# facebookresearch/hyperreel

Hardware: NVIDIA H100
Metric: Mrays/s at 65k-ray x 32-sample batch (higher is better)
Workload: dtype f32 (sample net bf16x3 split on wgmma, fp32 accumulate)

## Files before the change

### hyperreel_b200/csrc/hr_mlp_tc2.cu

```cuda
#include <cuda.h>
#include <cuda_bf16.h>

#include <cstdio>
#include <cstdlib>
#include <cstring>

#include "hr_encode.cuh"
#include "hr_handle.h"
#include "hr_tc_prims.cuh"

namespace hr {

namespace tc2 {
using namespace tc;

constexpr int NSTAGE = 4;
constexpr int STAGE_BYTES = 8192;
constexpr int KSTEP_BYTES = 4096;
constexpr int CONSUMERS = 2;
constexpr int NTHREADS = (CONSUMERS + 1) * 128;
constexpr int PRODUCER_REGS = 40;
constexpr int CONSUMER_REGS = 232;
static_assert(128 * PRODUCER_REGS + CONSUMERS * 128 * CONSUMER_REGS <= 65536, "register file");

constexpr int A_BYTES = 16 * KSTEP_BYTES;
constexpr int OFF_AHI = 0;
constexpr int OFF_ALO = OFF_AHI + A_BYTES;
constexpr int X_BYTES = 4 * KSTEP_BYTES;
constexpr int OFF_X = OFF_ALO + A_BYTES;
constexpr int OFF_B = OFF_X + 2 * X_BYTES;
constexpr int OFF_BAR = OFF_B + CONSUMERS * NSTAGE * STAGE_BYTES;
constexpr int SMEM_BYTES = OFF_BAR + 128;
static_assert(SMEM_BYTES <= 232448, "shared memory budget");

constexpr int BAR_FULL = 0;
constexpr int BAR_EMPTY = BAR_FULL + CONSUMERS * NSTAGE;
static_assert((BAR_EMPTY + CONSUMERS * NSTAGE) * 8 <= 128, "barrier block");

constexpr int NB_RET = 3;
constexpr int NB_WR = 5;
constexpr int NB_XW = 7;
constexpr int NB_XR = 9;

}

template <int W, bool SAVE, bool NARROW>
__global__ void __launch_bounds__(tc2::NTHREADS, 1)
mlp_tc2_kernel(const __grid_constant__ hr_config cfg, const __grid_constant__ MlpTcPack pk, const float* __restrict__ rays,
               float* __restrict__ heads, long long n_rays, float* __restrict__ rays_copy, const TrainSave sv) {
  using namespace tc2;
  constexpr int WH = W / 2;
  constexpr int NACC = WH / 2;
  constexpr int NK = W / 16;
  constexpr int NKH = NK / 2;
  constexpr int IMG_BYTES = WH * 64;
  constexpr int KPS = STAGE_BYTES / IMG_BYTES;
  static_assert(KPS * IMG_BYTES == STAGE_BYTES && NKH % KPS == 0 && NK * KSTEP_BYTES <= A_BYTES, "pass width");
  extern __shared__ __align__(128) uint8_t smem[];
  const uint32_t sbase = smem_u32(smem);
  const int tid = threadIdx.x, warp = tid >> 5, lane = tid & 31;
  auto bar = [&](int slot) -> uint32_t { return sbase + OFF_BAR + slot * 8; };

  {
    const char* w = reinterpret_cast<const char*>(pk.wpack);
    const long long lines = pk.wpack_bytes >> 7;
    for (long long i = (long long)blockIdx.x * NTHREADS + tid; i < lines; i += (long long)gridDim.x * NTHREADS)
      asm volatile("prefetch.global.L2 [%0];" ::"l"(w + i * 128));
  }
  for (int i = tid; i < (2 * X_BYTES) / 16; i += NTHREADS)
    reinterpret_cast<uint4*>(smem + OFF_X)[i] = make_uint4(0u, 0u, 0u, 0u);
  if (tid == 0) {
    for (int s = 0; s < CONSUMERS * NSTAGE; ++s) { mbar_init(bar(BAR_FULL + s), 1); mbar_init(bar(BAR_EMPTY + s), 1); }
    asm volatile("fence.mbarrier_init.release.cluster;" ::: "memory");
  }
  __syncthreads();

  const long long n_tiles = (n_rays + BM - 1) / BM;
  const int n_passes = pk.n_passes;
  const long long n_iters = ((long long)blockIdx.x < n_tiles) ? (n_tiles - 1 - blockIdx.x) / gridDim.x + 1 : 0;

  if (warp >= CONSUMERS * 4) {
    setmaxnreg_dec<PRODUCER_REGS>();
    const int g = warp - CONSUMERS * 4;
    if (g < CONSUMERS && lane == 0) {
      const long long half_bytes = pk.wpack_bytes / CONSUMERS;
      const int n_stages = (int)(half_bytes / STAGE_BYTES);
      const uint32_t full0 = bar(BAR_FULL + g * NSTAGE), empty0 = bar(BAR_EMPTY + g * NSTAGE);
      const uint32_t ring = sbase + OFF_B + (uint32_t)(g * NSTAGE * STAGE_BYTES);
      uint32_t stage = 0, phase = 0;
      for (long long iter = 0; iter < n_iters; ++iter) {
        const uint8_t* src = reinterpret_cast<const uint8_t*>(pk.wpack) + g * half_bytes;
        for (int i = 0; i < n_stages; ++i) {
          mbar_wait(empty0 + stage * 8, phase ^ 1);
          mbar_expect_tx(full0 + stage * 8, STAGE_BYTES);
          bulk_g2s(ring + stage * STAGE_BYTES, src, STAGE_BYTES, full0 + stage * 8);
          src += STAGE_BYTES;
          if (++stage == NSTAGE) { stage = 0; phase ^= 1; }
        }
      }
    }
    return;
  }

  setmaxnreg_inc<CONSUMER_REGS>();
  const int wg = warp >> 2;
  const int wt = tid & 127;
  const int rowq = (warp & 3) * 16 + (lane >> 2);
  const int q2 = (lane & 3) * 2;
  const int col0 = wg * WH;
  const int in_chunks = pk.in_chunks;
  const int L = cfg.mlp_layers;
  const uint32_t x_lo_off = (uint32_t)(2 * in_chunks * KSTEP_BYTES);
  const uint32_t full0 = bar(BAR_FULL + wg * NSTAGE), empty0 = bar(BAR_EMPTY + wg * NSTAGE);
  const uint32_t ring = sbase + OFF_B + (uint32_t)(wg * NSTAGE * STAGE_BYTES);
  const bool vec_ok = ((reinterpret_cast<uintptr_t>(rays) | reinterpret_cast<uintptr_t>(rays_copy)) & 15) == 0;
  int x_last = 0;
  for (int p = 0; p < n_passes; ++p)
    if (pk.passes[p].first_chunk == 0) x_last = p;
  uint32_t stage = 0, phase = 0;
  int pend = -1;

  float acc[2][NACC];

  auto stage_begin = [&]() {
    mbar_wait(full0 + stage * 8, phase);
    wgmma_fence();
    acc_fence(acc[0]);
    acc_fence(acc[1]);
  };
  auto stage_end = [&]() {
    wgmma_commit();
    acc_fence(acc[0]);
    acc_fence(acc[1]);
    wgmma_wait<1>();
    if (pend >= 0 && wt == 0) mbar_arrive(empty0 + pend * 8);
    pend = (int)stage;
    if (++stage == NSTAGE) { stage = 0; phase ^= 1; }
  };
  auto b_img = [&](int sub) -> uint32_t { return ring + stage * STAGE_BYTES + (uint32_t)sub * IMG_BYTES; };
  auto kstep = [&](uint32_t a, uint32_t a_lo, uint32_t b, uint32_t scale) {
    const uint64_t bh = gmma_desc(b, WH * 16, 128), bl = gmma_desc(b + WH * 32, WH * 16, 128);
    const uint64_t ah0 = gmma_desc(a, 2048, 128), ah1 = gmma_desc(a + 1024, 2048, 128);
    const uint64_t al0 = gmma_desc(a + a_lo, 2048, 128), al1 = gmma_desc(a + a_lo + 1024, 2048, 128);
    wgmma_ss(acc[0], ah0, bh, scale);
    wgmma_ss(acc[1], ah1, bh, scale);
    wgmma_ss(acc[0], al0, bh, 1u);
    wgmma_ss(acc[1], al1, bh, 1u);
    wgmma_ss(acc[0], ah0, bl, 1u);
    wgmma_ss(acc[1], ah1, bl, 1u);
  };
  auto run_pass = [&](const TcPass& P, bool fresh, bool x_ret, bool ret) {
    int ki = 0;
    if (P.first_chunk == 0) {
      for (; ki < 2 * in_chunks; ki += KPS) {
        stage_begin();
#pragma unroll
        for (int sub = 0; sub < KPS; ++sub)
          kstep(sbase + OFF_X + (uint32_t)(ki + sub) * KSTEP_BYTES, x_lo_off, b_img(sub), (ki + sub) != 0 ? 1u : 0u);
        stage_end();
      }
    }
    if (P.first_chunk + P.n_chunks > in_chunks) {
      const uint32_t scale0 = ki != 0 ? 1u : 0u;
#pragma unroll
      for (int kk = 0; kk < NK; ++kk) {
        if (kk % KPS == 0) {
          if (fresh && kk == (wg == 0 ? NKH : 0)) {
            if (wg == 0) pair_arrive(NB_WR + 0);
            pair_wait(NB_WR + (wg ^ 1));
          }
          stage_begin();
        }
        kstep(sbase + OFF_AHI + (uint32_t)kk * KSTEP_BYTES, OFF_ALO - OFF_AHI, b_img(kk % KPS), kk != 0 ? 1u : scale0);
        if (kk % KPS == KPS - 1) {
          stage_end();
          if (x_ret && kk == KPS - 1) pair_arrive(NB_XR + wg);
          if (ret && wg == 1 && kk == NKH + KPS - 1) pair_arrive(NB_RET + 1);
        }
      }
    }
  };
  auto drain = [&]() {
    wgmma_wait<0>();
    acc_fence(acc[0]);
    acc_fence(acc[1]);
    if (pend >= 0 && wt == 0) mbar_arrive(empty0 + pend * 8);
    pend = -1;
  };
  const int st_row = (warp & 3) * 16 + 8 * ((lane >> 3) & 1) + (lane & 7);
  const uint32_t st_off = ks_slot(st_row, lane >> 4);
  auto store_hidden = [&](const float* bias, int layer, long long tile) {
#pragma unroll
    for (int kk = 0; kk < NKH; ++kk) {
      float2 b[2];
#pragma unroll
      for (int jj = 0; jj < 2; ++jj) b[jj] = __ldg(reinterpret_cast<const float2*>(bias + col0 + 8 * (2 * kk + jj) + q2));
#pragma unroll
      for (int m = 0; m < 2; ++m) {
        uint32_t hi[4], lo[4];
#pragma unroll
        for (int jj = 0; jj < 2; ++jj) {
          const int j = 2 * kk + jj, k = col0 + 8 * j + q2;
#pragma unroll
          for (int h = 0; h < 2; ++h) {
            float t0 = acc[m][4 * j + 2 * h] + b[jj].x, t1 = acc[m][4 * j + 2 * h + 1] + b[jj].y;
            t0 = fmaxf(t0, t0 * cfg.leaky_slope);
            t1 = fmaxf(t1, t1 * cfg.leaky_slope);
            split2(t0, t1, hi[2 * jj + h], lo[2 * jj + h]);
            if constexpr (SAVE) {
              const long long ray = tile * BM + 64 * m + rowq + 8 * h;
              if (ray < n_rays) *reinterpret_cast<float2*>(sv.act + layer * sv.act_stride + ray * W + k) = make_float2(t0, t1);
            }
          }
        }
        const uint32_t a = sbase + st_off + (uint32_t)m * 1024u + (uint32_t)(wg * NKH + kk) * KSTEP_BYTES;
        stmatrix_x4(a + OFF_AHI, hi);
        stmatrix_x4(a + OFF_ALO, lo);
      }
    }
  };
  auto encode = [&](long long tile, bool after_x) {
    if (after_x) pair_wait(NB_XR + (wg ^ 1));
    const int r = wg * 64 + (wt & 63), part = wt >> 6;
    const long long ray = tile * BM + r;
    auto put = [&](int k, float val) {
      if constexpr (SAVE) {
        if (ray < n_rays) sv.enc[ray * sv.ld_enc + k] = val;
      }
      const __nv_bfloat16 hi = __float2bfloat16_rn(val);
      const __nv_bfloat16 lo = __float2bfloat16_rn(val - __bfloat162float(hi));
      const uint32_t off = (uint32_t)(k >> 4) * KSTEP_BYTES + ks_slot(r, (k >> 3) & 1) + (uint32_t)(k & 7) * 2u;
      *reinterpret_cast<__nv_bfloat16*>(smem + OFF_X + off) = hi;
      *reinterpret_cast<__nv_bfloat16*>(smem + OFF_X + x_lo_off + off) = lo;
    };
    if (ray < n_rays) {
      float rbuf[16];
      const float* src = rays + ray * cfg.c_in;
      if (cfg.c_in == 8 && vec_ok) {
        const float4 a = *reinterpret_cast<const float4*>(src), b = *reinterpret_cast<const float4*>(src + 4);
        rbuf[0] = a.x; rbuf[1] = a.y; rbuf[2] = a.z; rbuf[3] = a.w; rbuf[4] = b.x; rbuf[5] = b.y; rbuf[6] = b.z; rbuf[7] = b.w;
        if (rays_copy != nullptr && part == 0) {
          float4* dst = reinterpret_cast<float4*>(rays_copy + ray * 8);
          dst[0] = a; dst[1] = b;
        }
      } else {
        for (int i = 0; i < cfg.c_in; ++i) rbuf[i] = src[i];
        if (rays_copy != nullptr && part == 0)
          for (int i = 0; i < cfg.c_in; ++i) rays_copy[ray * cfg.c_in + i] = rbuf[i];
      }
      encode_ray_features(cfg, rbuf, part, 2, put);
      if constexpr (SAVE) {
        if (part == 0)
          for (int k = cfg.mlp_in; k < sv.ld_enc; ++k) sv.enc[ray * sv.ld_enc + k] = 0.0f;
      }
    } else if (part == 0) {
      for (int k = 0; k < cfg.mlp_in; ++k) put(k, 0.0f);
    }
    fence_async_smem();
    wg_sync(1 + wg);
    pair_arrive(NB_XW + wg);
  };

  for (long long iter = 0; iter < n_iters; ++iter) {
    const long long tile = iter * gridDim.x + blockIdx.x;
    const bool more = iter + 1 < n_iters;
    if (iter == 0) encode(tile, false);
    pair_wait(NB_XW + (wg ^ 1));
    for (int p = 0; p < n_passes; ++p) {
      const TcPass& P = pk.passes[p];
      const bool reads_a = P.first_chunk + P.n_chunks > in_chunks;
      const bool hidden = p < L - 1;
      const bool ret = reads_a && (hidden || (p == n_passes - 1 && more));
      const bool x_ret = p == x_last && more;
      run_pass(P, reads_a && P.wait_a != 0, x_ret, ret);
      drain();
      if (x_ret && !reads_a) pair_arrive(NB_XR + wg);
      if (ret && wg == 0) pair_arrive(NB_RET + 0);
      if (hidden) {
        wg_sync(1 + wg);
        if (p > 0 || iter > 0) pair_wait(NB_RET + (wg ^ 1));
        store_hidden(pk.bias + P.bias_off, p, tile);
        fence_async_smem();
        wg_sync(1 + wg);
        if (wg == 1) pair_arrive(NB_WR + 1);
      } else {
        const float* bias = pk.bias + P.bias_off;
        if constexpr (SAVE) {
#pragma unroll
          for (int m = 0; m < 2; ++m)
#pragma unroll
            for (int h = 0; h < 2; ++h) {
              const long long ray = tile * BM + 64 * m + rowq + 8 * h;
              if (ray >= n_rays) continue;
              float* row = heads + ray * cfg.mlp_out;
#pragma unroll
              for (int j = 0; j < WH / 8; ++j) {
                const int c = col0 + 8 * j + q2;
                if (P.out_col0 + c < cfg.mlp_out) {
                  const float2 b = __ldg(reinterpret_cast<const float2*>(bias + c));
                  const int c0 = P.out_col0 + c, c1 = c0 + 1, S = cfg.n_samples;
                  row[(c0 % S) * cfg.head_stride + c0 / S] = acc[m][4 * j + 2 * h] + b.x;
                  if (c1 < cfg.mlp_out) row[(c1 % S) * cfg.head_stride + c1 / S] = acc[m][4 * j + 2 * h + 1] + b.y;
                }
              }
            }
        } else if constexpr (NARROW) {
          const bool pairs = (cfg.mlp_out % 2) == 0 && (reinterpret_cast<uintptr_t>(heads) & 7) == 0;
#pragma unroll
          for (int j = 0; j < WH / 8; ++j) {
            const int c = col0 + 8 * j + q2, c0 = P.out_col0 + c;
            const float2 b = __ldg(reinterpret_cast<const float2*>(bias + c));
#pragma unroll
            for (int m = 0; m < 2; ++m)
#pragma unroll
              for (int h = 0; h < 2; ++h) {
                const long long ray = tile * BM + 64 * m + rowq + 8 * h;
                if (ray >= n_rays || c0 >= cfg.mlp_out) continue;
                float* dst = heads + ray * cfg.mlp_out + c0;
                const float v0 = acc[m][4 * j + 2 * h] + b.x, v1 = acc[m][4 * j + 2 * h + 1] + b.y;
                if (pairs) {
                  *reinterpret_cast<float2*>(dst) = make_float2(v0, v1);
                } else {
                  dst[0] = v0;
                  if (c0 + 1 < cfg.mlp_out) dst[1] = v1;
                }
              }
          }
        } else {
          const bool odd = (lane & 1) != 0;
#pragma unroll
          for (int jp = 0; jp < WH / 16; ++jp) {
            const int j = 2 * jp, c = col0 + 8 * j + q2;
            const float2 b0 = __ldg(reinterpret_cast<const float2*>(bias + c));
            const float2 b1 = __ldg(reinterpret_cast<const float2*>(bias + c + 8));
#pragma unroll
            for (int m = 0; m < 2; ++m)
#pragma unroll
              for (int h = 0; h < 2; ++h) {
                const float2 v0 = make_float2(acc[m][4 * j + 2 * h] + b0.x, acc[m][4 * j + 2 * h + 1] + b0.y);
                const float2 v1 = make_float2(acc[m][4 * j + 4 + 2 * h] + b1.x, acc[m][4 * j + 4 + 2 * h + 1] + b1.y);
                const float2 send = odd ? v0 : v1;
                const float2 recv = make_float2(__shfl_xor_sync(0xffffffffu, send.x, 1), __shfl_xor_sync(0xffffffffu, send.y, 1));
                const int c4 = odd ? c + 6 : c;
                const long long ray = tile * BM + 64 * m + rowq + 8 * h;
                if (ray < n_rays && P.out_col0 + c4 < cfg.mlp_out)
                  *reinterpret_cast<float4*>(heads + ray * cfg.mlp_out + P.out_col0 + c4) =
                      odd ? make_float4(recv.x, recv.y, v1.x, v1.y) : make_float4(v0.x, v0.y, recv.x, recv.y);
              }
          }
        }
      }
      if (x_ret) encode(tile + gridDim.x, true);
    }
  }
}

int pack_mlp_tc2(SampleNet& net, const float* const* w_dev, const float* const* b_dev, cudaStream_t st) {
  const hr_config& c = net.cfg;
  MlpTcPack& pk = net.tc;
  size_t& alloc_bytes = net.tc_alloc_bytes;
  int& alloc_bias = net.tc_alloc_bias;
  const int W = c.mlp_width;
  if (W != 128 && W != 256) return hr_fail("tensor-core sample net: hidden width must be 128 or 256 (got %d)", W);
  if (c.mlp_in > 64) return hr_fail("tensor-core sample net: encoded input wider than 64 features (%d)", c.mlp_in);
  const int in_chunks = (c.mlp_in + 31) / 32;
  const int L = c.mlp_layers;
  MlpTcPack np_{};
  np_.in_chunks = in_chunks;
  int np = 0, bias_off = 0;
  size_t bytes = 0;
  for (int l = 0; l < L; ++l) {
    const bool last = (l == L - 1);
    const int out = last ? c.mlp_out : W;
    const int n_parts = (out + W - 1) / W;
    for (int part = 0; part < n_parts; ++part) {
      if (np >= HR_TC_MAX_PASSES) return hr_fail("tensor-core sample net: too many passes (%d output columns)", c.mlp_out);
      TcPass& P = np_.passes[np++];
      const bool reads_input = (l == 0 || l == c.mlp_skip);
      P.layer = l;
      P.n = W;
      P.first_chunk = reads_input ? 0 : in_chunks;
      P.n_chunks = (l == 0) ? in_chunks : (W / 32 + (reads_input ? in_chunks : 0));
      P.bias_off = bias_off;
      P.is_final = last ? 1 : 0;
      P.out_col0 = part * W;
      P.wait_a = (part == 0) ? 1 : 0;
      bias_off += P.n;
      bytes += (size_t)P.n_chunks * 2 * P.n * 64;
    }
  }
  np_.n_passes = np;
  np_.bias_count = bias_off;
  np_.wpack_bytes = (long long)bytes;
  if (alloc_bytes != bytes || alloc_bias != bias_off || !pk.wpack) {
    if (pk.wpack) cudaFree(const_cast<void*>(pk.wpack));
    if (pk.bias) cudaFree(const_cast<float*>(pk.bias));
    pk.wpack = nullptr; pk.bias = nullptr;
    alloc_bytes = 0; alloc_bias = 0;
    void* wp = nullptr; float* bp = nullptr;
    cudaError_t e = cudaMalloc(&wp, bytes);
    if (e != cudaSuccess) return hr_fail("cudaMalloc(tc weights %zu): %s", bytes, cudaGetErrorString(e));
    e = cudaMalloc((void**)&bp, (size_t)bias_off * sizeof(float));
    if (e != cudaSuccess) { cudaFree(wp); return hr_fail("cudaMalloc(tc bias): %s", cudaGetErrorString(e)); }
    np_.wpack = wp; np_.bias = bp;
    alloc_bytes = bytes; alloc_bias = bias_off;
    for (int narrow = 0; narrow < 2 && e == cudaSuccess; ++narrow) {
      auto kern = (W == 256) ? (narrow ? mlp_tc2_kernel<256, false, true> : mlp_tc2_kernel<256, false, false>)
                             : (narrow ? mlp_tc2_kernel<128, false, true> : mlp_tc2_kernel<128, false, false>);
      e = cudaFuncSetAttribute(kern, cudaFuncAttributeMaxDynamicSharedMemorySize, tc2::SMEM_BYTES);
    }
    if (e != cudaSuccess) return hr_fail("cudaFuncSetAttribute(mlp_tc2_kernel): %s", cudaGetErrorString(e));
  } else {
    np_.wpack = pk.wpack; np_.bias = pk.bias;
  }
  pk = np_;
  uint8_t* wp = (uint8_t*)const_cast<void*>(pk.wpack);
  float* bp = const_cast<float*>(pk.bias);
  const int WH = W / 2;
  for (int half = 0; half < 2; ++half) {
    size_t off = (size_t)half * (bytes / 2);
    for (int p = 0; p < np; ++p) {
      const TcPass& P = pk.passes[p];
      const int l = P.layer;
      const bool last = (l == L - 1), skip = (l == c.mlp_skip), first = (l == 0);
      const int in_src = first ? c.mlp_in : (skip ? c.mlp_in + W : W);
      launch_pack_tc_pass(w_dev[l], b_dev[l], wp + off, bp + P.bias_off + half * WH, WH, P.first_chunk, P.n_chunks, in_src,
                          c.mlp_in, skip ? 1 : 0, in_chunks, last ? c.mlp_out : W, last ? c.n_samples : 0, c.head_stride,
                          P.out_col0 + half * WH, st);
      off += (size_t)P.n_chunks * 2 * WH * 64;
    }
  }
  cudaError_t e = cudaGetLastError();
  if (e != cudaSuccess) return hr_fail("tc pack launch failed: %s", cudaGetErrorString(e));
  return 0;
}

void free_mlp_tc2(SampleNet& net) {
  if (net.tc.wpack) cudaFree(const_cast<void*>(net.tc.wpack));
  if (net.tc.bias) cudaFree(const_cast<float*>(net.tc.bias));
  net.tc.wpack = nullptr; net.tc.bias = nullptr;
  net.tc_alloc_bytes = 0; net.tc_alloc_bias = 0;
}

cudaError_t launch_mlp_tc2(const hr_config& cfg, const MlpTcPack& pk, const float* rays, float* heads, long long n, int num_sms,
                           cudaStream_t stream, float* rays_copy) {
  long long tiles = (n + tc::BM - 1) / tc::BM;
  int grid = (int)(tiles < num_sms ? tiles : num_sms);
  if (grid < 1) grid = 1;
  const bool narrow = (cfg.mlp_out % 4) != 0 || ((uintptr_t)heads % 16) != 0;
  auto kern = cfg.mlp_width == 256 ? (narrow ? mlp_tc2_kernel<256, false, true> : mlp_tc2_kernel<256, false, false>)
                                   : (narrow ? mlp_tc2_kernel<128, false, true> : mlp_tc2_kernel<128, false, false>);
  if (cfg.mlp_width != 256 && cfg.mlp_width != 128) return cudaErrorInvalidValue;
  kern<<<grid, tc2::NTHREADS, tc2::SMEM_BYTES, stream>>>(cfg, pk, rays, heads, n, rays_copy, TrainSave{});
  return cudaGetLastError();
}

cudaError_t launch_mlp_tc2_train(const hr_config& cfg, const MlpTcPack& pk, const float* rays, float* heads, long long n,
                                 int num_sms, cudaStream_t stream, const TrainSave& sv) {
  long long tiles = (n + tc::BM - 1) / tc::BM;
  int grid = (int)(tiles < num_sms ? tiles : num_sms);
  if (grid < 1) grid = 1;
  auto kern = cfg.mlp_width == 256 ? mlp_tc2_kernel<256, true, false> : mlp_tc2_kernel<128, true, false>;
  if (cfg.mlp_width != 256 && cfg.mlp_width != 128) return cudaErrorInvalidValue;
  cudaError_t e = cudaFuncSetAttribute(kern, cudaFuncAttributeMaxDynamicSharedMemorySize, tc2::SMEM_BYTES);
  if (e != cudaSuccess) return e;
  kern<<<grid, tc2::NTHREADS, tc2::SMEM_BYTES, stream>>>(cfg, pk, rays, heads, n, nullptr, sv);
  return cudaGetLastError();
}

}
```

### hyperreel_b200/csrc/hr_tc_prims.cuh

```cuda
#pragma once
#include <cuda.h>
#include <cuda_bf16.h>
#include <stdint.h>

namespace hr {
namespace tc {

constexpr int BM = 128;

__device__ __forceinline__ uint32_t smem_u32(const void* p) { return (uint32_t)__cvta_generic_to_shared(p); }

__device__ __forceinline__ void mbar_init(uint32_t bar, uint32_t count) {
  asm volatile("mbarrier.init.shared::cta.b64 [%0], %1;" ::"r"(bar), "r"(count) : "memory");
}
__device__ __forceinline__ void mbar_arrive(uint32_t bar) {
  asm volatile("{\n\t.reg .b64 st;\n\tmbarrier.arrive.shared::cta.b64 st, [%0];\n\t}" ::"r"(bar) : "memory");
}
__device__ __forceinline__ void mbar_expect_tx(uint32_t bar, uint32_t bytes) {
  asm volatile("{\n\t.reg .b64 st;\n\tmbarrier.arrive.expect_tx.shared::cta.b64 st, [%0], %1;\n\t}" ::"r"(bar), "r"(bytes)
               : "memory");
}
__device__ __forceinline__ void mbar_wait(uint32_t bar, uint32_t parity) {
  asm volatile(
      "{\n\t"
      ".reg .pred p;\n\t"
      "WAIT_LOOP:\n\t"
      "mbarrier.try_wait.parity.shared::cta.b64 p, [%0], %1;\n\t"
      "@p bra DONE;\n\t"
      "bra WAIT_LOOP;\n\t"
      "DONE:\n\t"
      "}" ::"r"(bar), "r"(parity)
      : "memory");
}
__device__ __forceinline__ void bulk_g2s(uint32_t dst, const void* src, uint32_t bytes, uint32_t bar) {
  asm volatile("cp.async.bulk.shared::cluster.global.mbarrier::complete_tx::bytes [%0], [%1], %2, [%3];" ::"r"(dst), "l"(src),
               "r"(bytes), "r"(bar)
               : "memory");
}
__device__ __forceinline__ void fence_async_smem() { asm volatile("fence.proxy.async.shared::cta;" ::: "memory"); }
__device__ __forceinline__ void wg_sync(int id) { asm volatile("bar.sync %0, 128;" ::"r"(id) : "memory"); }
__device__ __forceinline__ void pair_arrive(int id) { asm volatile("bar.arrive %0, 256;" ::"r"(id) : "memory"); }
__device__ __forceinline__ void pair_wait(int id) { asm volatile("bar.sync %0, 256;" ::"r"(id) : "memory"); }

__device__ __forceinline__ uint64_t gmma_desc(uint32_t saddr, uint32_t lbo_bytes, uint32_t sbo_bytes) {
  uint64_t d = 0;
  d |= (uint64_t)((saddr & 0x3FFFF) >> 4);
  d |= (uint64_t)((lbo_bytes >> 4) & 0x3FFF) << 16;
  d |= (uint64_t)((sbo_bytes >> 4) & 0x3FFF) << 32;
  return d;
}

__device__ __forceinline__ void wgmma_fence() { asm volatile("wgmma.fence.sync.aligned;" ::: "memory"); }
__device__ __forceinline__ void wgmma_commit() { asm volatile("wgmma.commit_group.sync.aligned;" ::: "memory"); }
template <int N>
__device__ __forceinline__ void wgmma_wait() {
  asm volatile("wgmma.wait_group.sync.aligned %0;" ::"n"(N) : "memory");
}
template <int N>
__device__ __forceinline__ void acc_fence(float (&d)[N]) {
#pragma unroll
  for (int i = 0; i < N; ++i) asm volatile("" : "+f"(d[i])::"memory");
}
template <int R>
__device__ __forceinline__ void setmaxnreg_dec() { asm volatile("setmaxnreg.dec.sync.aligned.u32 %0;" ::"n"(R)); }
template <int R>
__device__ __forceinline__ void setmaxnreg_inc() { asm volatile("setmaxnreg.inc.sync.aligned.u32 %0;" ::"n"(R)); }

__device__ __forceinline__ void wgmma_ss(float (&d)[32], uint64_t adesc, uint64_t bdesc, uint32_t accumulate) {
  asm volatile(
      "{\n\t"
      ".reg .pred p;\n\t"
      "setp.ne.b32 p, %34, 0;\n\t"
      "wgmma.mma_async.sync.aligned.m64n64k16.f32.bf16.bf16 "
      "{"
      "%0, %1, %2, %3, %4, %5, %6, %7, %8, %9, %10, %11, %12, %13, %14, %15, %16, %17, %18, %19, %20, %21, %22, "
      "%23, %24, %25, %26, %27, %28, %29, %30, %31"
      "}, %32, %33, p, 1, 1, 0, 0;\n\t"
      "}"
      : "+f"(d[0]), "+f"(d[1]), "+f"(d[2]), "+f"(d[3]), "+f"(d[4]), "+f"(d[5]), "+f"(d[6]), "+f"(d[7]),
        "+f"(d[8]), "+f"(d[9]), "+f"(d[10]), "+f"(d[11]), "+f"(d[12]), "+f"(d[13]), "+f"(d[14]), "+f"(d[15]),
        "+f"(d[16]), "+f"(d[17]), "+f"(d[18]), "+f"(d[19]), "+f"(d[20]), "+f"(d[21]), "+f"(d[22]), "+f"(d[23]),
        "+f"(d[24]), "+f"(d[25]), "+f"(d[26]), "+f"(d[27]), "+f"(d[28]), "+f"(d[29]), "+f"(d[30]), "+f"(d[31])
      : "l"(adesc), "l"(bdesc), "r"(accumulate));
}

__device__ __forceinline__ void wgmma_ss(float (&d)[64], uint64_t adesc, uint64_t bdesc, uint32_t accumulate) {
  asm volatile(
      "{\n\t"
      ".reg .pred p;\n\t"
      "setp.ne.b32 p, %66, 0;\n\t"
      "wgmma.mma_async.sync.aligned.m64n128k16.f32.bf16.bf16 "
      "{"
      "%0, %1, %2, %3, %4, %5, %6, %7, %8, %9, %10, %11, %12, %13, %14, %15, %16, %17, %18, %19, %20, %21, %22, "
      "%23, %24, %25, %26, %27, %28, %29, %30, %31, %32, %33, %34, %35, %36, %37, %38, %39, %40, %41, %42, %43, "
      "%44, %45, %46, %47, %48, %49, %50, %51, %52, %53, %54, %55, %56, %57, %58, %59, %60, %61, %62, %63"
      "}, %64, %65, p, 1, 1, 0, 0;\n\t"
      "}"
      : "+f"(d[0]), "+f"(d[1]), "+f"(d[2]), "+f"(d[3]), "+f"(d[4]), "+f"(d[5]), "+f"(d[6]), "+f"(d[7]),
        "+f"(d[8]), "+f"(d[9]), "+f"(d[10]), "+f"(d[11]), "+f"(d[12]), "+f"(d[13]), "+f"(d[14]), "+f"(d[15]),
        "+f"(d[16]), "+f"(d[17]), "+f"(d[18]), "+f"(d[19]), "+f"(d[20]), "+f"(d[21]), "+f"(d[22]), "+f"(d[23]),
        "+f"(d[24]), "+f"(d[25]), "+f"(d[26]), "+f"(d[27]), "+f"(d[28]), "+f"(d[29]), "+f"(d[30]), "+f"(d[31]),
        "+f"(d[32]), "+f"(d[33]), "+f"(d[34]), "+f"(d[35]), "+f"(d[36]), "+f"(d[37]), "+f"(d[38]), "+f"(d[39]),
        "+f"(d[40]), "+f"(d[41]), "+f"(d[42]), "+f"(d[43]), "+f"(d[44]), "+f"(d[45]), "+f"(d[46]), "+f"(d[47]),
        "+f"(d[48]), "+f"(d[49]), "+f"(d[50]), "+f"(d[51]), "+f"(d[52]), "+f"(d[53]), "+f"(d[54]), "+f"(d[55]),
        "+f"(d[56]), "+f"(d[57]), "+f"(d[58]), "+f"(d[59]), "+f"(d[60]), "+f"(d[61]), "+f"(d[62]), "+f"(d[63])
      : "l"(adesc), "l"(bdesc), "r"(accumulate));
}

__device__ __forceinline__ void stmatrix_x4(uint32_t addr, const uint32_t (&r)[4]) {
  asm volatile("stmatrix.sync.aligned.m8n8.x4.shared.b16 [%0], {%1, %2, %3, %4};" ::"r"(addr), "r"(r[0]), "r"(r[1]), "r"(r[2]),
               "r"(r[3])
               : "memory");
}

__device__ __forceinline__ uint32_t ks_slot(int row, int kg) { return (uint32_t)((kg * 16 + (row >> 3)) * 128 + (row & 7) * 16); }

__device__ __forceinline__ void split2(float x0, float x1, uint32_t& hi, uint32_t& lo) {
  __nv_bfloat162 hh = __floats2bfloat162_rn(x0, x1);
  __nv_bfloat162 ll = __floats2bfloat162_rn(x0 - __low2float(hh), x1 - __high2float(hh));
  hi = *reinterpret_cast<uint32_t*>(&hh);
  lo = *reinterpret_cast<uint32_t*>(&ll);
}

}

void launch_pack_tc_pass(const float* W, const float* b, uint8_t* dst, float* bias_dst, int n, int first_chunk, int n_chunks,
                         int in_src, int mlp_in, int is_skip, int in_chunks, int out_rows, int perm_S, int perm_stride,
                         int out_col0, cudaStream_t st);
}
```

Baseline: 155.3.

## Move ray encoding into dedicated encoder warps of the producer warpgroup

Result: faster. 157.6, median of 6 (+1.5%).

```diff
diff --git a/hyperreel_b200/csrc/hr_mlp_tc2.cu b/hyperreel_b200/csrc/hr_mlp_tc2.cu
--- a/hyperreel_b200/csrc/hr_mlp_tc2.cu
+++ b/hyperreel_b200/csrc/hr_mlp_tc2.cu
@@ -19,9 +19,11 @@
 constexpr int KSTEP_BYTES = 4096;
 constexpr int CONSUMERS = 2;
 constexpr int NTHREADS = (CONSUMERS + 1) * 128;
-constexpr int PRODUCER_REGS = 40;
-constexpr int CONSUMER_REGS = 232;
-static_assert(128 * PRODUCER_REGS + CONSUMERS * 128 * CONSUMER_REGS <= 65536, "register file");
+constexpr int ENCODERS = 64;
+constexpr int PRODUCER_REGS = 56;
+constexpr int CONSUMER_REGS = 224;
+constexpr int LAUNCH_REGS = 168;
+static_assert(128 * PRODUCER_REGS + CONSUMERS * 128 * CONSUMER_REGS <= NTHREADS * LAUNCH_REGS, "register file");
 
 constexpr int A_BYTES = 16 * KSTEP_BYTES;
 constexpr int OFF_AHI = 0;
@@ -39,9 +41,51 @@
 
 constexpr int NB_RET = 3;
 constexpr int NB_WR = 5;
-constexpr int NB_XW = 7;
-constexpr int NB_XR = 9;
-
+constexpr int NB_XFULL = 7;
+constexpr int NB_XFREE = 9;
+constexpr int XFULL_THREADS = ENCODERS + 128;
+constexpr int XFREE_THREADS = CONSUMERS * 128 + ENCODERS;
+
+}
+
+template <bool SAVE>
+__device__ __forceinline__ void encode_row(const hr_config& cfg, const float* __restrict__ rays, long long n_rays,
+                                           float* __restrict__ rays_copy, const TrainSave& sv, uint8_t* smem,
+                                           uint32_t x_lo_off, bool vec_ok, long long tile, int r) {
+  using namespace tc2;
+  const long long ray = tile * BM + r;
+  auto put = [&](int k, float val) {
+    if constexpr (SAVE) {
+      if (ray < n_rays) sv.enc[ray * sv.ld_enc + k] = val;
+    }
+    const __nv_bfloat16 hi = __float2bfloat16_rn(val);
+    const __nv_bfloat16 lo = __float2bfloat16_rn(val - __bfloat162float(hi));
+    const uint32_t off = (uint32_t)(k >> 4) * KSTEP_BYTES + ks_slot(r, (k >> 3) & 1) + (uint32_t)(k & 7) * 2u;
+    *reinterpret_cast<__nv_bfloat16*>(smem + OFF_X + off) = hi;
+    *reinterpret_cast<__nv_bfloat16*>(smem + OFF_X + x_lo_off + off) = lo;
+  };
+  if (ray < n_rays) {
+    float rbuf[16];
+    const float* src = rays + ray * cfg.c_in;
+    if (cfg.c_in == 8 && vec_ok) {
+      const float4 a = *reinterpret_cast<const float4*>(src), b = *reinterpret_cast<const float4*>(src + 4);
+      rbuf[0] = a.x; rbuf[1] = a.y; rbuf[2] = a.z; rbuf[3] = a.w; rbuf[4] = b.x; rbuf[5] = b.y; rbuf[6] = b.z; rbuf[7] = b.w;
+      if (rays_copy != nullptr) {
+        float4* dst = reinterpret_cast<float4*>(rays_copy + ray * 8);
+        dst[0] = a; dst[1] = b;
+      }
+    } else {
+      for (int i = 0; i < cfg.c_in; ++i) rbuf[i] = src[i];
+      if (rays_copy != nullptr)
+        for (int i = 0; i < cfg.c_in; ++i) rays_copy[ray * cfg.c_in + i] = rbuf[i];
+    }
+    encode_ray_features(cfg, rbuf, 0, 1, put);
+    if constexpr (SAVE) {
+      for (int k = cfg.mlp_in; k < sv.ld_enc; ++k) sv.enc[ray * sv.ld_enc + k] = 0.0f;
+    }
+  } else {
+    for (int k = 0; k < cfg.mlp_in; ++k) put(k, 0.0f);
+  }
 }
 
 template <int W, bool SAVE, bool NARROW>
@@ -79,10 +123,23 @@
   const int n_passes = pk.n_passes;
   const long long n_iters = ((long long)blockIdx.x < n_tiles) ? (n_tiles - 1 - blockIdx.x) / gridDim.x + 1 : 0;
 
+  const int in_chunks = pk.in_chunks;
+  const uint32_t x_lo_off = (uint32_t)(2 * in_chunks * KSTEP_BYTES);
   if (warp >= CONSUMERS * 4) {
     setmaxnreg_dec<PRODUCER_REGS>();
     const int g = warp - CONSUMERS * 4;
-    if (g < CONSUMERS && lane == 0) {
+    if (g >= CONSUMERS) {
+      const int et = tid - (NTHREADS - ENCODERS);
+      const bool vec_ok = ((reinterpret_cast<uintptr_t>(rays) | reinterpret_cast<uintptr_t>(rays_copy)) & 15) == 0;
+      for (long long iter = 0; iter < n_iters; ++iter) {
+        const long long tile = iter * gridDim.x + blockIdx.x;
+        if (iter > 0) bar_sync_n(NB_XFREE, XFREE_THREADS);
+        for (int r = et; r < BM; r += ENCODERS)
+          encode_row<SAVE>(cfg, rays, n_rays, rays_copy, sv, smem, x_lo_off, vec_ok, tile, r);
+        fence_async_smem();
+        for (int c = 0; c < CONSUMERS; ++c) bar_arrive_n(NB_XFULL + c, XFULL_THREADS);
+      }
+    } else if (lane == 0) {
       const long long half_bytes = pk.wpack_bytes / CONSUMERS;
       const int n_stages = (int)(half_bytes / STAGE_BYTES);
       const uint32_t full0 = bar(BAR_FULL + g * NSTAGE), empty0 = bar(BAR_EMPTY + g * NSTAGE);
@@ -108,12 +165,9 @@
   const int rowq = (warp & 3) * 16 + (lane >> 2);
   const int q2 = (lane & 3) * 2;
   const int col0 = wg * WH;
-  const int in_chunks = pk.in_chunks;
   const int L = cfg.mlp_layers;
-  const uint32_t x_lo_off = (uint32_t)(2 * in_chunks * KSTEP_BYTES);
   const uint32_t full0 = bar(BAR_FULL + wg * NSTAGE), empty0 = bar(BAR_EMPTY + wg * NSTAGE);
   const uint32_t ring = sbase + OFF_B + (uint32_t)(wg * NSTAGE * STAGE_BYTES);
-  const bool vec_ok = ((reinterpret_cast<uintptr_t>(rays) | reinterpret_cast<uintptr_t>(rays_copy)) & 15) == 0;
   int x_last = 0;
   for (int p = 0; p < n_passes; ++p)
     if (pk.passes[p].first_chunk == 0) x_last = p;
@@ -174,7 +228,7 @@
         kstep(sbase + OFF_AHI + (uint32_t)kk * KSTEP_BYTES, OFF_ALO - OFF_AHI, b_img(kk % KPS), kk != 0 ? 1u : scale0);
         if (kk % KPS == KPS - 1) {
           stage_end();
-          if (x_ret && kk == KPS - 1) pair_arrive(NB_XR + wg);
+          if (x_ret && kk == KPS - 1) bar_arrive_n(NB_XFREE, XFREE_THREADS);
           if (ret && wg == 1 && kk == NKH + KPS - 1) pair_arrive(NB_RET + 1);
         }
       }
@@ -219,53 +273,10 @@
       }
     }
   };
-  auto encode = [&](long long tile, bool after_x) {
-    if (after_x) pair_wait(NB_XR + (wg ^ 1));
-    const int r = wg * 64 + (wt & 63), part = wt >> 6;
-    const long long ray = tile * BM + r;
-    auto put = [&](int k, float val) {
-      if constexpr (SAVE) {
-        if (ray < n_rays) sv.enc[ray * sv.ld_enc + k] = val;
-      }
-      const __nv_bfloat16 hi = __float2bfloat16_rn(val);
-      const __nv_bfloat16 lo = __float2bfloat16_rn(val - __bfloat162float(hi));
-      const uint32_t off = (uint32_t)(k >> 4) * KSTEP_BYTES + ks_slot(r, (k >> 3) & 1) + (uint32_t)(k & 7) * 2u;
-      *reinterpret_cast<__nv_bfloat16*>(smem + OFF_X + off) = hi;
-      *reinterpret_cast<__nv_bfloat16*>(smem + OFF_X + x_lo_off + off) = lo;
-    };
-    if (ray < n_rays) {
-      float rbuf[16];
-      const float* src = rays + ray * cfg.c_in;
-      if (cfg.c_in == 8 && vec_ok) {
-        const float4 a = *reinterpret_cast<const float4*>(src), b = *reinterpret_cast<const float4*>(src + 4);
-        rbuf[0] = a.x; rbuf[1] = a.y; rbuf[2] = a.z; rbuf[3] = a.w; rbuf[4] = b.x; rbuf[5] = b.y; rbuf[6] = b.z; rbuf[7] = b.w;
-        if (rays_copy != nullptr && part == 0) {
-          float4* dst = reinterpret_cast<float4*>(rays_copy + ray * 8);
-          dst[0] = a; dst[1] = b;
-        }
-      } else {
-        for (int i = 0; i < cfg.c_in; ++i) rbuf[i] = src[i];
-        if (rays_copy != nullptr && part == 0)
-          for (int i = 0; i < cfg.c_in; ++i) rays_copy[ray * cfg.c_in + i] = rbuf[i];
-      }
-      encode_ray_features(cfg, rbuf, part, 2, put);
-      if constexpr (SAVE) {
-        if (part == 0)
-          for (int k = cfg.mlp_in; k < sv.ld_enc; ++k) sv.enc[ray * sv.ld_enc + k] = 0.0f;
-      }
-    } else if (part == 0) {
-      for (int k = 0; k < cfg.mlp_in; ++k) put(k, 0.0f);
-    }
-    fence_async_smem();
-    wg_sync(1 + wg);
-    pair_arrive(NB_XW + wg);
-  };
-
   for (long long iter = 0; iter < n_iters; ++iter) {
     const long long tile = iter * gridDim.x + blockIdx.x;
     const bool more = iter + 1 < n_iters;
-    if (iter == 0) encode(tile, false);
-    pair_wait(NB_XW + (wg ^ 1));
+    bar_sync_n(NB_XFULL + wg, XFULL_THREADS);
     for (int p = 0; p < n_passes; ++p) {
       const TcPass& P = pk.passes[p];
       const bool reads_a = P.first_chunk + P.n_chunks > in_chunks;
@@ -274,7 +285,7 @@
       const bool x_ret = p == x_last && more;
       run_pass(P, reads_a && P.wait_a != 0, x_ret, ret);
       drain();
-      if (x_ret && !reads_a) pair_arrive(NB_XR + wg);
+      if (x_ret && !reads_a) bar_arrive_n(NB_XFREE, XFREE_THREADS);
       if (ret && wg == 0) pair_arrive(NB_RET + 0);
       if (hidden) {
         wg_sync(1 + wg);
@@ -350,7 +361,6 @@
           }
         }
       }
-      if (x_ret) encode(tile + gridDim.x, true);
     }
   }
 }
diff --git a/hyperreel_b200/csrc/hr_tc_prims.cuh b/hyperreel_b200/csrc/hr_tc_prims.cuh
--- a/hyperreel_b200/csrc/hr_tc_prims.cuh
+++ b/hyperreel_b200/csrc/hr_tc_prims.cuh
@@ -41,6 +41,8 @@
 __device__ __forceinline__ void wg_sync(int id) { asm volatile("bar.sync %0, 128;" ::"r"(id) : "memory"); }
 __device__ __forceinline__ void pair_arrive(int id) { asm volatile("bar.arrive %0, 256;" ::"r"(id) : "memory"); }
 __device__ __forceinline__ void pair_wait(int id) { asm volatile("bar.sync %0, 256;" ::"r"(id) : "memory"); }
+__device__ __forceinline__ void bar_arrive_n(int id, int n) { asm volatile("bar.arrive %0, %1;" ::"r"(id), "r"(n) : "memory"); }
+__device__ __forceinline__ void bar_sync_n(int id, int n) { asm volatile("bar.sync %0, %1;" ::"r"(id), "r"(n) : "memory"); }
 
 __device__ __forceinline__ uint64_t gmma_desc(uint32_t saddr, uint32_t lbo_bytes, uint32_t sbo_bytes) {
   uint64_t d = 0;
```
